# google-research/corenet

Hardware: AMD Instinct MI355X
Metric: voxels/sec fwd+bwd @128^3 (higher is better)
Workload: dtype bf16x3 (the convolutions of decoder stages 3-6 and the encoder's 3x3 convolutions -- forward of stages 4-5, data gradient of all -- multiply operands split into two bf16 terms: three bf16 MFMAs per product, fp32 accumulation, 16 mantissa bits, ~3e-6 relative per layer; tensors, everything else and t

## Files before the change

### corenet_amd/_lib.py

```python
from __future__ import annotations

import ctypes as C
import os
from typing import Optional

import torch as t

_HERE = os.path.dirname(os.path.abspath(__file__))
TOOLS_LIB_PATH = os.path.join(os.path.dirname(_HERE), "tools", "_build", "libcorenet_hip_tools.so")
PROBE_LIB_PATH = os.path.join(os.path.dirname(_HERE), "tools", "_build", "libcrn_probe.so")
LIB_PATH = os.environ.get("CORENET_HIP_LIB", TOOLS_LIB_PATH if os.environ.get("CRN_TOOLS_LIB") == "1" else
                          os.path.join(_HERE, "lib", "libcorenet_hip.so"))

c_i32p = C.POINTER(C.c_int32)
c_f32p = C.c_void_p
vp = C.c_void_p
i64 = C.c_int64
i32 = C.c_int
f32 = C.c_float
sz = C.c_size_t


class CrnTapBoxes(C.Structure):
  _fields_ = [("n_groups", C.c_int32), ("c_groups", C.c_int32), ("n_box", (C.c_int8 * 6) * 8),
# ... 104 lines not shown
    "crn_scatter_f32": [vp, vp, vp, i64, i32, vp],
    "crn_bias_grad": [vp, i32, i32, i64, i64, vp, i32, vp, sz, vp],
    "crn_batch_renorm_stats": [vp, i32, i32, i64, i64, i32, vp, vp, vp, vp, vp, f32, f32, i32,
                               vp, vp, vp, vp, sz, vp],
    "crn_batch_renorm_stats_tail": [vp, i32, i32, i64, i64, vp, vp, vp, vp, vp, f32, f32, i32, vp, vp, vp, vp, sz,
                                    vp, vp, vp, i64, vp, i64, vp, i64, i32, vp, i32, vp],
    "crn_batch_renorm_bwd_head": [vp, i64, vp, i64, vp, i64, vp, i64, vp, i64, i32, i32, i64, vp, vp, vp, vp, vp, i64,
                                  vp, vp, i32, vp, i32, vp, sz, vp, i32, vp],
    "crn_batch_renorm_bwd": [vp, i64, vp, i64, i32, i32, i64, i32, i32, vp, vp, vp, vp, vp, i64,
                             vp, vp, i32, vp, i32, vp, sz, vp],
    "crn_affine_add_relu": [vp, vp, vp, vp, vp, vp, i32, i32, i64, i64, i64, vp, i64, vp, i64, i32, vp],
    "crn_relu_bwd_add": [vp, vp, vp, i32, i32, i64, i64, i64, i64, vp, i64, vp],
    "crn_preprocess_caffe": [vp, i32, i32, i32, vp, vp],
    "crn_stem_conv_fwd": [vp, i32, i32, i32, vp, vp, vp, vp, sz, vp],
    "crn_stem_conv_wgrad": [vp, i32, i32, i32, vp, vp, vp],
    "crn_batch_renorm_finalize": [vp, i32, i32, C.c_double, vp, vp, vp, vp, vp, f32, f32, vp, vp, vp, vp],
    "crn_bn_relu_maxpool_fwd": [vp, vp, vp, i32, i32, i32, i32, vp, vp, vp],
    "crn_bn_relu_maxpool_bwd": [vp, vp, i32, i32, i32, i32, vp, vp],
    "crn_relu_mean_fwd": [vp, i32, i32, i64, i64, vp, vp],
    "crn_relu_mean_bwd": [vp, vp, i32, i32, i64, i64, vp, i64, i32, vp],
    "crn_linear_fwd": [vp, vp, vp, i32, i32, i32, vp, i32, vp],
    "crn_linear_bwd": [vp, vp, vp, i32, i32, i32, i32, vp, vp, vp, vp],
    "crn_stride2_gather": [vp, vp, i32, i32, i32, i32, i32, i32, vp],
    "crn_stride2_scatter": [vp, vp, i32, i32, i32, i32, i32, i32, vp],
    "crn_fill_offset_channels": [vp, i32, i64, i64, i32, vp, vp],
    "crn_decoder_inputs": [vp, vp, i32, i32, C.POINTER(C.c_float), vp, vp, vp],
    "crn_ray_sample_fwd": [vp, i64, i64, i64, i32, i32, i32, i32, vp, vp, vp, i64, i32, i32, i32, vp],
    "crn_ray_sample_bwd": [vp, i64, i32, i32, i32, i32, i32, vp, vp, vp, i64, i32, i32, i32, vp],
    "crn_ray_sample_fwd_idx": [vp, i64, i64, i64, i32, i32, i32, i32, vp, vp, vp, i64, i32, i32, i32, vp, vp],
    "crn_ray_project": [vp, vp, i32, i32, i32, i32, i32, i32, vp, vp],
# ... 193 lines not shown
```

### corenet_amd/backend.py

```python
from __future__ import annotations

import ctypes as C
from typing import Optional

import torch as t

from corenet_amd import _lib
from corenet_amd._lib import CrnInTransform, CrnView, ptr
from corenet_amd.views import View, space_to_depth_view, view_of

_DTYPE_CODE = {t.float32: 0, t.uint8: 1, t.int32: 2, t.float64: 3, t.int64: 4, t.int16: 5, t.int8: 6}


def _cview(v: View) -> CrnView:
  base = v.storage.data_ptr() + 4 * (v.offset - v.storage.storage_offset())
  c = v.__dict__.get("_crn")
  if c is None or c[0] != base:
    c = (base, CrnView(base, v.B, v.C, v.D, v.H, v.W, v.sB, v.sC, ptr(v.chan_off), v.sD, v.sH, v.sW))
    object.__setattr__(v, "_crn", c)
  return c[1]


class Transform:
  __slots__ = ("scale", "shift", "pre_relu", "post_relu")
# ... 333 lines not shown
  def relu_bwd_add(self, dy, y_pre, dy2, B, Cn, S, sB_dy, sB_pre, sB_dy2, dx, sB_dx):
    self.lib.crn_relu_bwd_add(ptr(dy), ptr(y_pre), ptr(dy2), B, Cn, S, sB_dy, sB_pre, sB_dy2,
                              ptr(dx), sB_dx, _lib.stream())

  def preprocess(self, img_u8, out):
    B, _, H, W = img_u8.shape
    self.lib.crn_preprocess_caffe(ptr(img_u8), B, H, W, ptr(out), _lib.stream())

  def maxpool_fwd(self, x, scale, shift, B, Cn, H, W, y, argmax):
    self.lib.crn_bn_relu_maxpool_fwd(ptr(x), ptr(scale), ptr(shift), B, Cn, H, W, ptr(y), ptr(argmax),
                                     _lib.stream())

  def maxpool_bwd(self, dy, argmax, B, Cn, H, W, dx):
    self.lib.crn_bn_relu_maxpool_bwd(ptr(dy), ptr(argmax), B, Cn, H, W, ptr(dx), _lib.stream())

  def relu_mean_fwd(self, x_pre, B, Cn, S, sB, avg):
    self.lib.crn_relu_mean_fwd(ptr(x_pre), B, Cn, S, sB, ptr(avg), _lib.stream())

  def relu_mean_bwd(self, x_pre, davg, B, Cn, S, sB, dx, sB_dx, accumulate=False):
    self.lib.crn_relu_mean_bwd(ptr(x_pre), ptr(davg), B, Cn, S, sB, ptr(dx), sB_dx, int(accumulate),
                               _lib.stream())

  def linear_fwd(self, x, w, bias, B, K, N, y, ldy):
    self.lib.crn_linear_fwd(ptr(x), ptr(w), ptr(bias), B, K, N, ptr(y), ldy, _lib.stream())

  def linear_bwd(self, x, w, dy, lddy, B, K, N, dx, dw, db):
    self.lib.crn_linear_bwd(ptr(x), ptr(w), ptr(dy), lddy, B, K, N, ptr(dx), ptr(dw), ptr(db),
                            _lib.stream())

  def stride2_gather(self, x, y):
# ... 202 lines not shown
```

### corenet_amd/build.py

```python
import os
import subprocess
import sys
from concurrent.futures import ThreadPoolExecutor

HERE = os.path.dirname(os.path.abspath(__file__))
CSRC = os.path.join(HERE, "csrc")
LIBDIR = os.path.join(HERE, "lib")
LIB = os.path.join(LIBDIR, "libcorenet_hip.so")
SOURCES = ["conv_igemm.hip", "splitk.hip", "conv_bf3.hip", "conv_e2d.hip", "batch_renorm.hip", "ray_sample.hip", "misc_ops.hip", "losses.hip", "fill_voxels.hip",
           "voxelize.hip", "comm_rccl.hip", "stem_conv.hip", "convt_par.hip", "fill_voxels_cpu.cpp", "marching_cubes.hip",
           "marching_cubes_cpu.cpp", "render.hip", "render_cpu.cpp", "point_metrics.hip", "point_metrics_cpu.cpp",
           "eval_labels.hip", "eval_labels_cpu.cpp", "voxel_components.hip", "voxel_components_cpu.cpp",
           "voxel_distance.hip", "voxel_distance_cpu.cpp", "voxel_visibility.hip", "voxel_visibility_cpu.cpp",
           "voxel_overlap.hip", "voxel_overlap_cpu.cpp"]
CONV_CONFIGS = [(8, 1), (4, 2), (4, 1), (2, 4), (2, 2), (2, 1), (1, 4), (1, 2), (1, 1)]
FLAGS = ["--offload-arch=gfx950", "-O3", "-std=c++17", "-fPIC", "-munsafe-fp-atomics",
         "-ffp-contract=off", "-Wno-unused-result"]


HOST_FLAGS = ["-O3", "-std=c++17", "-fPIC", "-ffp-contract=off", "-pthread"]


def _stale(obj, src):
  if not os.path.exists(obj):
    return True
  m = os.path.getmtime(obj)
  deps = [src, os.path.join(CSRC, "crn_common.h"), os.path.join(CSRC, "splitk.h"), os.path.join(CSRC, "conv_kernels.h"), os.path.join(CSRC, "bf3_common.h"),
          os.path.join(CSRC, "mc_tables.h"), os.path.join(CSRC, "marching_cubes_common.h"),
          os.path.join(CSRC, "render_common.h"), os.path.join(CSRC, "point_metrics_common.h"),
          os.path.join(CSRC, "eval_labels_common.h"), os.path.join(CSRC, "voxel_components_common.h"),
          os.path.join(CSRC, "voxel_distance_common.h"), os.path.join(CSRC, "voxel_visibility_common.h"),
          os.path.join(CSRC, "voxel_overlap_common.h"),
          os.path.join(HERE, "..", "include", "corenet_hip.h")]
  return any(os.path.getmtime(d) > m for d in deps)


def build(verbose=True, force=False):
  os.makedirs(LIBDIR, exist_ok=True)
  hipcc = os.environ.get("HIPCC", "/opt/rocm/bin/hipcc")
  objs, jobs = [], []
  for s in SOURCES:
    src = os.path.join(CSRC, s)
    obj = os.path.join(LIBDIR, os.path.splitext(s)[0] + ".o")
    objs.append(obj)
    if force or _stale(obj, src):
      flags = FLAGS if s.endswith(".hip") else HOST_FLAGS
      jobs.append([hipcc] + flags + ["-c", src, "-o", obj])
# ... 64 lines not shown
```

### corenet_amd/csrc/batch_renorm.hip

```cpp
#include "crn_common.h"
#include <cstdlib>
#include <algorithm>
#include <type_traits>

namespace {

constexpr int kThreads = 256;

struct Slice { int64_t s0, s1; };
__device__ __forceinline__ Slice block_slice(int64_t S) {
  int64_t chunk = (S + gridDim.x - 1) / gridDim.x;
  chunk = (chunk + 3) & ~(int64_t)3;
  Slice r;
  r.s0 = (int64_t)blockIdx.x * chunk;
  r.s1 = min(S, r.s0 + chunk);
  return r;
}

template <bool VEC, typename F4, typename F1>
__device__ __forceinline__ void for_slice(Slice sl, F4 f4, F1 f1) {
  if (VEC) {
#pragma unroll 4
    for (int64_t s = sl.s0 + (int64_t)threadIdx.x * 4; s + 3 < sl.s1; s += (int64_t)kThreads * 4) f4(s);
    const int64_t nfull = (sl.s1 > sl.s0) ? ((sl.s1 - sl.s0) & ~(int64_t)3) : 0;
// ... 259 lines not shown
        if (tail.y) {
          if (tail.relu) {
#pragma unroll
            for (int i = 0; i < 4; ++i) q[i] = fmaxf(q[i], 0.f);
          }
          *reinterpret_cast<f32x4*>(tail.y + (int64_t)b * tail.sBy + o) = q;
          int64_t o2;
          if (tail.y2 && bn_stride2_offset(c, s4, tail.W, tail.W2, tail.H2, o2))
            *reinterpret_cast<f32x2*>(tail.y2 + (int64_t)b * tail.sBy2 + o2) = (f32x2){q[0], q[2]};
        }
      }
    }
  }
}

struct BnBwdChannel { float sc, sh, mu, rstd; };
__device__ __forceinline__ BnBwdChannel bn_bwd_channel(int c, int C, const float* scale, const float* shift, const float* saved) {
  return BnBwdChannel{scale[c], shift[c], saved[c], saved[C + c]};
}

__device__ __forceinline__ void bn_bwd_acc(float x, float g, int pre_relu, int post_relu, BnBwdChannel ch, double& s1, double& s2) {
  if (pre_relu) x = fmaxf(x, 0.f);
  if (post_relu && !(x * ch.sc + ch.sh > 0.f)) g = 0.f;
  s1 += (double)g;
  s2 += (double)g * (double)((x - ch.mu) * ch.rstd);
}

__device__ __forceinline__ float bn_bwd_dx(float xr, float g, int pre_relu, int post_relu, BnBwdChannel ch, float k, float mg, float mgx) {
  const float x = pre_relu ? fmaxf(xr, 0.f) : xr;
  if (post_relu && !(x * ch.sc + ch.sh > 0.f)) g = 0.f;
  float o = k * (g - mg - (x - ch.mu) * ch.rstd * mgx);
  if (pre_relu && !(xr > 0.f)) o = 0.f;
  return o;
}

struct BnAffineGrad { float dg, db; };
__device__ __forceinline__ BnAffineGrad bn_bwd_close(double s1, double s2, double count, float r, float d, float* sm) {
  sm[0] = (float)(s1 / count); sm[1] = (float)(s2 / count);
  return BnAffineGrad{(float)(r * s2 + d * s1), (float)s1};
}
__device__ __forceinline__ void bn_bwd_store_grad(BnAffineGrad g, int c, float* dgamma, float* dbeta, int accumulate) {
  if (accumulate) { dgamma[c] += g.dg; dbeta[c] += g.db; } else { dgamma[c] = g.dg; dbeta[c] = g.db; }
}

__device__ __forceinline__ float bn_block_sum_f32(float v, float* redf) {
  const float w = crn_wave_sum(v);
  if ((threadIdx.x & 63) == 0) redf[threadIdx.x >> 6] = w;
  __syncthreads();
  float tsum = 0.f;
  if (threadIdx.x == 0)
    for (int i = 0; i < kThreads / 64; ++i) tsum += redf[i];
  return tsum;
}

struct BnHead { const float* g; int64_t sBg; const float* act; int64_t sBact; const float* g2; int64_t sBg2;
                const float* gc; int64_t sBgc; int W, W2, H2; };
template <int NV, bool HEAD = false>
__global__ __launch_bounds__(kThreads) void bn_owner_bwd_reg_kernel(
    const float* x, int64_t sBx, const float* dy, int64_t sBdy, int B, int S4, int C, int pre_relu,
// ... 85 lines not shown
    int post_relu, const float* scale, const float* shift, const float* saved, double* ws, float* dsum,
    int ndsum, const float* part, int splits) {
  __shared__ double red[kThreads / 64];
  const int c = blockIdx.y, b = blockIdx.z;
  if (dsum && c < ndsum && blockIdx.x == 0 && b == 0 && threadIdx.x == 0) dsum[c] = 0.f;
  const float* px = x + (int64_t)b * sBx + (int64_t)c * S;
  const BnPendingRow<PEND> pg = bn_pending_row<PEND>(dy, sBdy, part, splits, gridDim.z, C, S, b, c);
  const BnBwdChannel ch = bn_bwd_channel(c, C, scale, shift, saved);
  double s1 = 0.0, s2 = 0.0;
  auto one = [&](float xv, float gv) { bn_bwd_acc(xv, gv, pre_relu, post_relu, ch, s1, s2); };
  for_slice<VEC>(block_slice(S),
                 [&](int64_t s) { const f32x4 a = *reinterpret_cast<const f32x4*>(px + s);
                                  const f32x4 g = pg.at4(s);
                                  one(a.x, g.x); one(a.y, g.y); one(a.z, g.z); one(a.w, g.w); },
                 [&](int64_t s) { one(px[s], pg.at1(s)); });
  const double t1 = crn_block_sum(s1, red);
  const double t2 = crn_block_sum(s2, red);
  if (threadIdx.x == 0) {
    const int nparts = gridDim.x * gridDim.z;
    double* o = ws + ((int64_t)c * nparts + (int64_t)b * gridDim.x + blockIdx.x) * 2;
    o[0] = t1; o[1] = t2;
  }
}

template <bool VEC>
__global__ __launch_bounds__(kThreads) void bn_bwd_apply_kernel(
    const float* x, int64_t sBx, const float* dy, int64_t sBdy, int64_t S, int C, int pre_relu,
    int post_relu, const float* gamma, const float* scale, const float* shift, const float* saved,
    const double* ws, int nparts, double count, float* dx, int64_t sBdx, float* dgamma,
    float* dbeta, int accumulate, float* dsum, int ndsum) {
// ... 487 lines not shown
  float* const dsum_det = (dsum && ndsum > 0 && crn_deterministic()) ? dsum : nullptr;
  if (dsum_det && ws_bytes < (size_t)ndsum * ns * B * sizeof(double)) return CRN_ENOMEM;
  { const int rcf = crn_splitk_flush(st); if (rcf != CRN_OK) return rcf; }
  dim3 grid(ns, C, B);
  if (dsum_det) dsum = nullptr;
  with_bool(vec_ok(S, {sB_x, sB_dy, sB_dx}, {x, dy, dx}), [&](auto vec) {
    hipLaunchKernelGGL(bn_bwd_apply_kernel<decltype(vec)::value>, grid, dim3(kThreads), 0, st, x, sB_x, dy, sB_dy, S, C,
                       pre_relu, 0, gamma, scale, shift, saved, ws, nparts,
                       (double)B * (double)S, dx, sB_dx, dgamma, dbeta, accumulate, dsum, ndsum);
  });
  CRN_CHECK_LAUNCH();
  if (dsum_det) return bias_grad_ordered(dx, B, ndsum, S, sB_dx, ns, dsum_det, 0, ws, ws_bytes, st);
  return CRN_OK;
}

extern "C" int crn_batch_renorm_bwd_head(const float* x, int64_t sB_x, float* dy, int64_t sB_dy,
                                         const float* g, int64_t sB_g, const float* act, int64_t sB_act,
                                         const float* g2, int64_t sB_g2,
                                         int B, int C, int64_t S, const float* gamma, const float* scale,
                                         const float* shift, const float* saved, float* dx, int64_t sB_dx,
                                         float* dgamma, float* dbeta, int accumulate, float* dsum, int ndsum,
                                         double* ws, size_t ws_bytes, const float* g_compact, int W, crnStream stream) {
  if (!g || !act || !dy) return CRN_EINVAL;
  if (g_compact && (W < 1 || S % W || sB_g != (int64_t)C * S)) return CRN_EINVAL;
  const int H = g_compact ? (int)(S / W) : 0, H2 = (H + 1) / 2, W2 = (W + 1) / 2;
  const BnHead head{g, sB_g, act, sB_act, g2, sB_g2, g_compact, (int64_t)C * H2 * W2, W, W2, H2};
  return bn_bwd_impl(x, sB_x, dy, sB_dy, B, C, S, 0, 0, gamma, scale, shift, saved, dx, sB_dx, dgamma, dbeta,
                     accumulate, dsum, ndsum, ws, ws_bytes, stream, &head);
}

// ... 54 lines not shown
```

### corenet_amd/csrc/misc_ops.hip

```cpp
#include "crn_common.h"
#include <cstdlib>
#include <algorithm>
#include <cmath>

namespace {

__global__ void preprocess_kernel(const uint8_t* img, int64_t HW, float* out, int64_t total) {
  const int64_t e = blockIdx.x * (int64_t)blockDim.x + threadIdx.x;
  if (e >= total) return;
  const int64_t s = e % HW;
  const int c = (int)((e / HW) % 3);
  const int64_t b = e / (3 * HW);
  const float mean = c == 0 ? 103.939f : (c == 1 ? 116.779f : 123.68f);
  out[e] = (float)img[(b * 3 + (2 - c)) * HW + s] + mean;
}

__global__ void bn_relu_maxpool_fwd_kernel(const float* x, const float* scale, const float* shift,
                                           int C, int H, int W, int Ho, int Wo, float* y,
                                           int32_t* argmax, int64_t total) {
  const int64_t e = blockIdx.x * (int64_t)blockDim.x + threadIdx.x;
  if (e >= total) return;
  const int ow = (int)(e % Wo);
  const int oh = (int)((e / Wo) % Ho);
  const int64_t bc = e / ((int64_t)Wo * Ho);
// ... 15 lines not shown
    const float v = in ? fmaxf(raw[t9] * sc + sh, 0.f) : 0.f;
    const int idx = in ? ih * W + iw : -1;
    if (v > best) { best = v; bi = idx; }
  }
  y[e] = best;
  argmax[e] = (best > 0.f) ? bi : -1;
}

__global__ void bn_relu_maxpool_bwd_kernel(const float* dy, const int32_t* argmax, int H, int W,
                                           int Ho, int Wo, float* dx, int64_t total) {
  const int64_t e = blockIdx.x * (int64_t)blockDim.x + threadIdx.x;
  if (e >= total) return;
  const int iw = (int)(e % W);
  const int ih = (int)((e / W) % H);
  const int64_t bc = e / ((int64_t)W * H);
  const int idx = ih * W + iw;
  const float* g = dy + bc * (int64_t)Ho * Wo;
  const int32_t* am = argmax + bc * (int64_t)Ho * Wo;
  float s = 0.f;
  int amv[4];
  float gv[4];
#pragma unroll
  for (int q = 0; q < 4; ++q) {
    const int oh = min(ih / 2 + (q >> 1), Ho - 1), ow = min(iw / 2 + (q & 1), Wo - 1);
    amv[q] = am[oh * Wo + ow];
    gv[q] = g[oh * Wo + ow];
  }
#pragma unroll
  for (int q = 0; q < 4; ++q) {
    const int oh = ih / 2 + (q >> 1), ow = iw / 2 + (q & 1);
    const bool in = oh <= (ih + 1) / 2 && ow <= (iw + 1) / 2 && oh < Ho && ow < Wo;
    if (in && amv[q] == idx) s += gv[q];
  }
  dx[e] = s;
}

__global__ void relu_mean_fwd_kernel(const float* x, int C, int64_t S, int64_t sB, float* avg, int BC) {
  const int wid = (blockIdx.x * blockDim.x + threadIdx.x) >> 6, lane = threadIdx.x & 63;
  if (wid >= BC) return;
  const int b = wid / C, c = wid % C;
  const float* p = x + (int64_t)b * sB + (int64_t)c * S;
  double s = 0.0;
  for (int64_t i = lane; i < S; i += 64) s += (double)fmaxf(p[i], 0.f);
  s = crn_wave_sum(s);
  if (lane == 0) avg[wid] = (float)(s / (double)S);
}

__global__ void relu_mean_bwd_kernel(const float* x, const float* davg, int C, int64_t S, int64_t sB,
                                     float* dx, int64_t sBdx, int accumulate, int64_t total) {
// ... 535 lines not shown
```

### corenet_amd/csrc/stem_conv.hip

```cpp
#include "crn_common.h"
#include <cstdlib>
#include <algorithm>

namespace {

constexpr int kTH = 4, kTW = 32;
constexpr int kPH = 2 * kTH + 5;
constexpr int kPWf = 72;
constexpr int kPWg = 80;
constexpr int kKR = 3 * 7 * 8;
constexpr int kWP = 80;
constexpr int kDP = 84;
constexpr int kThreads = 256;

struct StemGeom {
  const float* img; const float* w; const float* bias; float* y; double* ws;
  const float* dy; float* dw;
  int B, H, W, H1, W1, tilesH, tilesW, ntiles;
};

__device__ __forceinline__ int packed_row(int c, int kh, int kw) {
  const int rh = (kh + 1) & 1, zh = (kh + 1) >> 1, rw = (kw + 1) & 1, zw = (kw + 1) >> 1;
  return (c * 4 + rh * 2 + rw) * 16 + zh * 4 + zw;
}

__device__ __forceinline__ void tile_of(const StemGeom& g, int tile, int& b, int& oh0, int& ow0) {
  const int tw = tile % g.tilesW; tile /= g.tilesW;
  const int th = tile % g.tilesH; b = tile / g.tilesH;
  oh0 = th * kTH; ow0 = tw * kTW;
}

template <int PW, int NE>
__device__ __forceinline__ void patch_load(const StemGeom& g, int b, int oh0, int ow0, int tid, float (&pv)[NE]) {
// ... 96 lines not shown
    for (int nb = 0; nb < 4; ++nb) {
      red[(wave * 64 + nb * 16 + i16) * 2 + 0] = s1[nb];
      red[(wave * 64 + nb * 16 + i16) * 2 + 1] = s2[nb];
    }
  }
  __syncthreads();
  if (tid < 64) {
    double a = 0.0, q = 0.0;
#pragma unroll
    for (int w = 0; w < 4; ++w) { a += (double)red[(w * 64 + tid) * 2]; q += (double)red[(w * 64 + tid) * 2 + 1]; }
    double* o = g.ws + ((int64_t)tid * gridDim.x + blockIdx.x) * 2;
    o[0] = a; o[1] = q;
  }
}

__global__ __launch_bounds__(kThreads) void stem_wgrad_kernel(StemGeom g) {
  __shared__ float pl[3 * kPH * kPWg];
  __shared__ float dl[kTH * kTW * kDP];
  crn_kernarg_touch(g);
  const int tid = threadIdx.x, lane = tid & 63, wave = tid >> 6, i16 = lane & 15, kk = lane >> 4;
  constexpr int NMB = (kKR + 15) / 16;
  int abase[NMB];
#pragma unroll
  for (int mb = 0; mb < NMB; ++mb) {
    const int T = min(mb * 16 + i16, kKR - 1);
    const int ck = T >> 3, kw = T & 7, c = ck / 7, kh = ck - c * 7;
    abase[mb] = (c * kPH + kh) * kPWg + kw + 2 * kk;
  }
  const int bbase = kk * kDP + wave * 16 + i16;
  f32x4 acc[NMB];
#pragma unroll
  for (int mb = 0; mb < NMB; ++mb) acc[mb] = (f32x4){0.f, 0.f, 0.f, 0.f};
  constexpr int NPE = (3 * kPH * kPWg + kThreads - 1) / kThreads;
  constexpr int NDV = kTH * kTW * 64 / 4 / kThreads;
  for (int tile = blockIdx.x; tile < g.ntiles; tile += gridDim.x) {
    int b, oh0, ow0;
    tile_of(g, tile, b, oh0, ow0);
    float pv[NPE];
    f32x4 dv[NDV];
    patch_load<kPWg>(g, b, oh0, ow0, tid, pv);
#pragma unroll
    for (int j = 0; j < NDV; ++j) {
      const int f = tid + j * kThreads;
      const int n = (f >> 9) * 16 + (f & 15), q4 = (f >> 4) & 31;
      const int oh = oh0 + (q4 >> 3), ow = ow0 + (q4 & 7) * 4;
      dv[j] = (oh < g.H1 && ow < g.W1) ? *reinterpret_cast<const f32x4*>(g.dy + ((int64_t)(b * 64 + n) * g.H1 + oh) * g.W1 + ow)
                                       : (f32x4){0.f, 0.f, 0.f, 0.f};
    }
    __syncthreads();
    patch_store<kPWg>(pl, tid, pv);
#pragma unroll
    for (int j = 0; j < NDV; ++j) {
      const int f = tid + j * kThreads;
      const int n = (f >> 9) * 16 + (f & 15), q4 = (f >> 4) & 31;
      float* d = dl + (q4 * 4) * kDP + n;
#pragma unroll
      for (int i = 0; i < 4; ++i) d[i * kDP] = dv[j][i];
    }
    __syncthreads();
#pragma unroll
    for (int q = 0; q < kTH * kTW / 4; ++q) {
      const int pr = q >> 3, qc = q & 7;
// ... 2 lines not shown
#pragma unroll
      for (int mb = 0; mb < NMB; ++mb)
        acc[mb] = __builtin_amdgcn_mfma_f32_16x16x4f32(pl[abase[mb] + ao], bv, acc[mb], 0, 0, 0);
    }
  }
  const int n = wave * 16 + i16;
#pragma unroll
  for (int mb = 0; mb < NMB; ++mb) {
#pragma unroll
    for (int r = 0; r < 4; ++r) {
      const int T = mb * 16 + kk * 4 + r;
      const int ck = T >> 3, kw = T & 7, c = ck / 7, kh = ck - c * 7;
      if (T < kKR && kw < 7) atomicAdd(g.dw + (int64_t)packed_row(c, kh, kw) * 64 + n, acc[mb][r]);
    }
  }
}

bool stem_shape_ok(int B, int H, int W) {
  return B >= 1 && H >= 8 && W >= 8 && (H & 1) == 0 && (W & 7) == 0 && (int64_t)B * H * W < ((int64_t)1 << 30);
}
StemGeom stem_geom(int B, int H, int W) {
  StemGeom g{};
  g.B = B; g.H = H; g.W = W; g.H1 = H / 2; g.W1 = W / 2;
  g.tilesH = crn_cdiv(g.H1, kTH); g.tilesW = crn_cdiv(g.W1, kTW);
  g.ntiles = B * g.tilesH * g.tilesW;
  return g;
}
}

extern "C" size_t crn_stem_conv_parts(int B, int H, int W) {
// ... 11 lines not shown
  if (stats_ws && ws_bytes < (size_t)64 * g.ntiles * 2 * sizeof(double)) return CRN_ENOMEM;
  hipLaunchKernelGGL(stem_fwd_kernel, dim3((unsigned)g.ntiles), dim3(kThreads), 0, (hipStream_t)stream, g);
  CRN_CHECK_LAUNCH();
  return CRN_OK;
}

extern "C" int crn_stem_conv_wgrad(const float* img, int B, int H, int W, const float* dy, float* dw_packed,
                                   crnStream stream) {
  CRN_ENTRY(stream);
  if (!img || !dy || !dw_packed || !stem_shape_ok(B, H, W)) return CRN_EINVAL;
  if (((uintptr_t)dy) & 15) return CRN_EINVAL;
  if (crn_deterministic()) return CRN_EINVAL;
  StemGeom g = stem_geom(B, H, W);
  g.img = img; g.dy = dy; g.dw = dw_packed;
  const int blocks = std::max(1, std::min(g.ntiles, 256));
  hipLaunchKernelGGL(stem_wgrad_kernel, dim3((unsigned)blocks), dim3(kThreads), 0, (hipStream_t)stream, g);
  CRN_CHECK_LAUNCH();
  return CRN_OK;
}
```

### corenet_amd/model/engine.py

```python
from __future__ import annotations

import dataclasses
import os
from typing import Dict, List, Optional, Tuple

import numpy as np
import torch as t

from corenet_amd import _lib
from corenet_amd import views as V
from corenet_amd.backend import Transform
from corenet_amd.model import conv_geometry as G

IMAGE_HW = (256, 256)


def check_image_hw(hw):
  H, W = int(hw[0]), int(hw[1])
  if H < 32 or W < 32 or H % 4 or W % 4 or H * W > 4096 * 4096:
    raise ValueError(f"corenet_amd.CoreNet: image batch of {H}x{W} pixels; this engine takes H and W that are multiples of 4 and >= 32 "
                     f"(256x256 in every shipped config)")
  return H, W
BN_EPS = 1e-3
BN_MOMENTUM = 0.01
# ... 547 lines not shown

def _no_exchange(grads: t.Tensor):
  """Bucket hook of a step without a gradient exchange."""


class Plan:

  def __init__(self, eng: Engine, B: int, hw=IMAGE_HW):
    self.eng, self.B = eng, B
    H, W = check_image_hw(hw)
    self.hw = (H, W)
    self.stem_hw = (H // 2, W // 2)
    parts = int(eng.be.lib.crn_stem_conv_parts(B, H, W)) if hasattr(eng.be, "stem_conv_fwd") else 0
    self.stem_fast = 0 < parts <= 4096
    self.dec_stats_fused = hasattr(eng.be, "conv_fwd_stats")
    self.pool_hw = (H // 4, W // 4)
    self.be = eng.be
    self.generation = 0
    self.graphs = {}
    self.eager_steps = 0
    self.eval_graph = None
    self.eval_eager = 0
    self._views = {}
    dev = eng.device
    self.dev = dev
    f = lambda *shape: t.zeros(*shape, dtype=eng.dtype, device=dev)
    self.in_image = t.zeros(B, 3, H, W, dtype=t.uint8, device=dev)
    self.in_v2s = f(B, 4, 4)
    self.in_off = f(B, 3)
    self.img = f(B, 3, H, W)
# ... 209 lines not shown
    g = cv.fwd
    math = self._math(cv, "wgrad")
    if self.stem_fast and cv.name == "encoder.stage1.conv.":
      math = "stem"
    if (self.eng.encoder_e2d and g.window in ((1, 1, 1), (1, 3, 3)) and self._wg2d_shape_ok(dy, g.window)
        and (cv.name.startswith("encoder.stage") and not cv.name.startswith("encoder.stage1")
             or cv.name.startswith("decoder.rt_skip"))):
      math = "bf16x3_2d"
    if cv.ct_kind == "par" and math == "bf16x3":
      math = "ct_par"
    return math

  def _launch_wgrad(self, cv: Conv, x: V.View, tr, dy: V.View, math: str, kw: dict):
    g = cv.fwd
    with _lib.roctx_range("wgrad " + cv.name):
      self.be.conv_wgrad(x, tr, dy, cv.gwf, g.npad, g.window, g.pad_lo, False, boxes=(g.n_boxes, g.c_boxes), math=math, **kw)

  def _wgrad(self, cv: Conv, x: V.View, tr, dy: V.View, here: bool = False):
    math = self._wgrad_math(cv, dy)
    kw = self._ximg_kw(math)
    if here:
      return self._launch_wgrad(cv, x, tr, dy, math, kw)
    if not self.overlap:
      return self._timed("wgrad " + cv.name, lambda: self._launch_wgrad(cv, x, tr, dy, math, kw))
    if cv.name.startswith("encoder."):
      self._wg_pending.append((cv, x, tr, dy, math, kw))
      return
    if self._handed_over:
      self._handed_over = False
      self._side_i = max(self._side_i, 1)
      ev = None
    else:
      ev = self._next_handover_event()
    with self._on_side(after=ev):
      self._launch_wgrad(cv, x, tr, dy, math, kw)
# ... 339 lines not shown
      t.cuda.current_stream().wait_event(self._skip_bwd_done)
    f5, g5 = self.feat["stage5"], self.gfeat["stage5"]
    last = self.blocks[-1]
    S5 = f5.shape[2] * f5.shape[3]
    be.relu_mean_bwd(f5, self.gavg, B, 2048, S5, f5.stride(0), last.gpre, 2048 * S5, False)
    be.affine_add_relu(last.gpre, None, None, g5, None, None, B, 2048, S5, 2048 * S5, g5.stride(0),
                       None, 0, last.gpre, 2048 * S5, False)
    g_in = None
    for blk in reversed(self.blocks):
      g_in = self._block_bwd(blk, g_in)
      self._flush_wgrads()
      if blk.prefix in GRAD_BUCKET_LABELS:
        self._grads_ready(blk.prefix, grad_hook)
    b1 = bn["encoder.stage1_part2.bn."]
    H1, W1 = self.stem_hw
    be.maxpool_bwd(g_in, self.p1_arg, B, 64, H1, W1, self.gy1)
    cs = cv["encoder.stage1.conv."]
    self._bn_bwd(b1, self.y1, self.gy1, self.gy1b, H1 * W1, False, False, bias_of=cs)
    self._wgrad(cs, self.s2d(self.img, 3, (1, 2, 2)), None, self.vw(self.gy1b))
    self._grads_ready("", grad_hook)
    self._join_side()
    if grad_hook is None:
      be.copy_tiles(eng.gpacked, eng.store.grads, eng.unpack_tiles, reverse=True)

  def _ray_bwd(self, k: int, g_out: t.Tensor):
    d, gm = self.dec[k], self.gsmap[k]
    ro, (hh, ww) = 2 * d.r, self.skip_hw[k]
    if self.ray_idx is not None:
      self.be.ray_sample_bwd_idx(g_out[:, d.cout:], g_out.stride(0), self.B, self.eng.skip_ch[k], ro, ro, ro,
                                 self.ray_idx[k], gm, gm.stride(0), hh, ww, False)
      return
    self.be.ray_sample_bwd(g_out[:, d.cout:], g_out.stride(0), self.B, self.eng.skip_ch[k], ro, ro, ro,
                           self.layer_mats[k - 2], self.offset, gm, gm.stride(0), hh, ww, False)

# ... 66 lines not shown
```

### include/corenet_hip.h

```cpp
#ifndef CORENET_HIP_H_
#define CORENET_HIP_H_

#include <stddef.h>
#include <stdint.h>

#ifdef __cplusplus
extern "C" {
#endif

#define CRN_OK 0
#define CRN_EINVAL (-1)
#define CRN_ENOMEM (-2)
#define CRN_ENOCONV (-3)

typedef void* crnStream;

typedef struct {
  float* base;
  int32_t B, C, D, H, W;
  int64_t sB, sC;
  const int32_t* chan_off;
  int32_t sD, sH, sW;
} crnView;

// ... 214 lines not shown

int crn_affine_add_relu(const float* x, const float* scale, const float* shift,
                        const float* r, const float* rscale, const float* rshift,
                        int B, int C, int64_t S, int64_t sB_x, int64_t sB_r,
                        float* y_pre, int64_t sB_pre, float* y, int64_t sB_y,
                        int relu, crnStream s);

int crn_relu_bwd_add(const float* dy, const float* y_pre, const float* dy2,
                     int B, int C, int64_t S, int64_t sB_dy, int64_t sB_pre, int64_t sB_dy2,
                     float* dx, int64_t sB_dx, crnStream s);

size_t crn_stem_conv_parts(int B, int H, int W);
int crn_stem_conv_fwd(const float* img, int B, int H, int W, const float* w_packed, const float* bias,
                      float* y, double* stats_ws , size_t ws_bytes, crnStream s);
int crn_stem_conv_wgrad(const float* img, int B, int H, int W, const float* dy, float* dw_packed, crnStream s);
int crn_batch_renorm_finalize(const double* ws, int nparts, int C, double count,
                              const float* gamma, const float* beta, float* running_mean, float* running_var,
                              const int64_t* nbt, float eps, float momentum,
                              float* scale, float* shift, float* saved, crnStream s);

int crn_preprocess_caffe(const uint8_t* img, int B, int H, int W, float* out, crnStream s);
int crn_bn_relu_maxpool_fwd(const float* x, const float* scale, const float* shift,
                            int B, int C, int H, int W, float* y, int32_t* argmax, crnStream s);
int crn_bn_relu_maxpool_bwd(const float* dy, const int32_t* argmax, int B, int C, int H, int W,
                            float* dx_bn , crnStream s);
int crn_relu_mean_fwd(const float* x_pre, int B, int C, int64_t S, int64_t sB, float* avg, crnStream s);
int crn_linear_fwd(const float* x, const float* w, const float* bias, int B, int K, int N,
                   float* y, int ldy, crnStream s);
int crn_linear_bwd(const float* x, const float* w, const float* dy, int lddy, int B, int K, int N,
                   float* dx, float* dw, float* db, crnStream s);
// ... 252 lines not shown
```

Measured before the change: 1.208 billion.

## Fuse stem maxpool backward with BN sums and BN-dx into stem wgrad

Replaces the three-step stem backward tail (maxpool backward, batch-renorm backward, stem weight-gradient) with two kernels. The maxpool backward now also accumulates the per-channel BN reduction sums. The stem wgrad kernel reduces those sums, applies the BN dx transform on the fly and also writes dgamma/dbeta and the bias gradient. This removes one full-resolution pass and the gy1b intermediate, at the cost of more complex kernels, an extra x load inside wgrad, and a non-deterministic path that is skipped under deterministic mode.

Result: no change. 1.198 billion (-0.9%).

```diff
diff --git a/corenet_amd/_lib.py b/corenet_amd/_lib.py
--- a/corenet_amd/_lib.py
+++ b/corenet_amd/_lib.py
@@ -142,6 +142,8 @@
     "crn_preprocess_caffe": [vp, i32, i32, i32, vp, vp],
     "crn_stem_conv_fwd": [vp, i32, i32, i32, vp, vp, vp, vp, sz, vp],
     "crn_stem_conv_wgrad": [vp, i32, i32, i32, vp, vp, vp],
+    "crn_maxpool_bwd_bn_sums": [vp, vp, i32, i32, i32, i32, vp, vp, vp, vp, vp, vp, i32, vp, sz, C.POINTER(C.c_int), vp],
+    "crn_stem_conv_wgrad_bn": [vp, i32, i32, i32, vp, vp, vp, vp, vp, sz, i32, vp, vp, vp, vp, i32, vp],
     "crn_batch_renorm_finalize": [vp, i32, i32, C.c_double, vp, vp, vp, vp, vp, f32, f32, vp, vp, vp, vp],
     "crn_bn_relu_maxpool_fwd": [vp, vp, vp, i32, i32, i32, i32, vp, vp, vp],
     "crn_bn_relu_maxpool_bwd": [vp, vp, i32, i32, i32, i32, vp, vp],
diff --git a/corenet_amd/backend.py b/corenet_amd/backend.py
--- a/corenet_amd/backend.py
+++ b/corenet_amd/backend.py
@@ -371,6 +371,24 @@
   def maxpool_bwd(self, dy, argmax, B, Cn, H, W, dx):
     self.lib.crn_bn_relu_maxpool_bwd(ptr(dy), ptr(argmax), B, Cn, H, W, ptr(dx), _lib.stream())
 
+  def maxpool_bwd_bn_sums(self, dy, argmax, B, Cn, H, W, x, scale, shift, saved, g, dsum=None, ndsum=0):
+    ws, n = self._bn_ws(Cn, x.device)
+    nparts = C.c_int(0)
+    self.lib.crn_maxpool_bwd_bn_sums(ptr(dy), ptr(argmax), B, Cn, H, W, ptr(x), ptr(scale), ptr(shift), ptr(saved), ptr(g),
+                                     ptr(dsum), int(ndsum), ptr(ws), n, C.byref(nparts), _lib.stream())
+    return ws, n, nparts.value
+
+  def stem_conv_wgrad_bn(self, img, gy, y, gamma, saved, sums, dw, dgamma, dbeta, dsum=None, ndsum=0) -> bool:
+    B, _, H, W = img.shape
+    ws, n, nparts = sums
+    rc = self.lib._crn_stem_conv_wgrad_bn(ptr(img), B, H, W, ptr(gy), ptr(y), ptr(gamma), ptr(saved), ptr(ws), n, nparts,
+                                          ptr(dw), ptr(dgamma), ptr(dbeta), ptr(dsum), int(ndsum), _lib.stream())
+    if rc == -1:
+      return False
+    if rc != 0:
+      raise _lib.HipError(f"crn_stem_conv_wgrad_bn failed with status {rc}")
+    return True
+
   def relu_mean_fwd(self, x_pre, B, Cn, S, sB, avg):
     self.lib.crn_relu_mean_fwd(ptr(x_pre), B, Cn, S, sB, ptr(avg), _lib.stream())
 
diff --git a/corenet_amd/build.py b/corenet_amd/build.py
--- a/corenet_amd/build.py
+++ b/corenet_amd/build.py
@@ -30,7 +30,7 @@
           os.path.join(CSRC, "render_common.h"), os.path.join(CSRC, "point_metrics_common.h"),
           os.path.join(CSRC, "eval_labels_common.h"), os.path.join(CSRC, "voxel_components_common.h"),
           os.path.join(CSRC, "voxel_distance_common.h"), os.path.join(CSRC, "voxel_visibility_common.h"),
-          os.path.join(CSRC, "voxel_overlap_common.h"),
+          os.path.join(CSRC, "voxel_overlap_common.h"), os.path.join(CSRC, "bn_bwd_common.h"),
           os.path.join(HERE, "..", "include", "corenet_hip.h")]
   return any(os.path.getmtime(d) > m for d in deps)
 
diff --git a/corenet_amd/csrc/batch_renorm.hip b/corenet_amd/csrc/batch_renorm.hip
--- a/corenet_amd/csrc/batch_renorm.hip
+++ b/corenet_amd/csrc/batch_renorm.hip
@@ -1,4 +1,5 @@
 #include "crn_common.h"
+#include "bn_bwd_common.h"
 #include <cstdlib>
 #include <algorithm>
 #include <type_traits>
@@ -297,35 +298,6 @@
   }
 }
 
-struct BnBwdChannel { float sc, sh, mu, rstd; };
-__device__ __forceinline__ BnBwdChannel bn_bwd_channel(int c, int C, const float* scale, const float* shift, const float* saved) {
-  return BnBwdChannel{scale[c], shift[c], saved[c], saved[C + c]};
-}
-
-__device__ __forceinline__ void bn_bwd_acc(float x, float g, int pre_relu, int post_relu, BnBwdChannel ch, double& s1, double& s2) {
-  if (pre_relu) x = fmaxf(x, 0.f);
-  if (post_relu && !(x * ch.sc + ch.sh > 0.f)) g = 0.f;
-  s1 += (double)g;
-  s2 += (double)g * (double)((x - ch.mu) * ch.rstd);
-}
-
-__device__ __forceinline__ float bn_bwd_dx(float xr, float g, int pre_relu, int post_relu, BnBwdChannel ch, float k, float mg, float mgx) {
-  const float x = pre_relu ? fmaxf(xr, 0.f) : xr;
-  if (post_relu && !(x * ch.sc + ch.sh > 0.f)) g = 0.f;
-  float o = k * (g - mg - (x - ch.mu) * ch.rstd * mgx);
-  if (pre_relu && !(xr > 0.f)) o = 0.f;
-  return o;
-}
-
-struct BnAffineGrad { float dg, db; };
-__device__ __forceinline__ BnAffineGrad bn_bwd_close(double s1, double s2, double count, float r, float d, float* sm) {
-  sm[0] = (float)(s1 / count); sm[1] = (float)(s2 / count);
-  return BnAffineGrad{(float)(r * s2 + d * s1), (float)s1};
-}
-__device__ __forceinline__ void bn_bwd_store_grad(BnAffineGrad g, int c, float* dgamma, float* dbeta, int accumulate) {
-  if (accumulate) { dgamma[c] += g.dg; dbeta[c] += g.db; } else { dgamma[c] = g.dg; dbeta[c] = g.db; }
-}
-
 __device__ __forceinline__ float bn_block_sum_f32(float v, float* redf) {
   const float w = crn_wave_sum(v);
   if ((threadIdx.x & 63) == 0) redf[threadIdx.x >> 6] = w;
@@ -441,6 +413,42 @@
                                   const f32x4 g = pg.at4(s);
                                   one(a.x, g.x); one(a.y, g.y); one(a.z, g.z); one(a.w, g.w); },
                  [&](int64_t s) { one(px[s], pg.at1(s)); });
+  const double t1 = crn_block_sum(s1, red);
+  const double t2 = crn_block_sum(s2, red);
+  if (threadIdx.x == 0) {
+    const int nparts = gridDim.x * gridDim.z;
+    double* o = ws + ((int64_t)c * nparts + (int64_t)b * gridDim.x + blockIdx.x) * 2;
+    o[0] = t1; o[1] = t2;
+  }
+}
+
+template <bool VEC>
+__global__ __launch_bounds__(kThreads) void maxpool_bwd_bn_sums_kernel(
+    const float* __restrict__ dyp, const int32_t* __restrict__ argmax, int H, int W, int Ho, int Wo, const float* __restrict__ x,
+    int C, const float* __restrict__ scale, const float* __restrict__ shift, const float* __restrict__ saved, float* __restrict__ g,
+    double* __restrict__ ws, float* __restrict__ dsum, int ndsum) {
+  __shared__ double red[kThreads / 64];
+  const int c = blockIdx.y, b = blockIdx.z;
+  const int64_t S = (int64_t)H * W, So = (int64_t)Ho * Wo, bc = (int64_t)b * C + c;
+  if (dsum && c < ndsum && blockIdx.x == 0 && b == 0 && threadIdx.x == 0) dsum[c] = 0.f;
+  const float* __restrict__ px = x + bc * S;
+  float* __restrict__ pg = g + bc * S;
+  const float* __restrict__ gp = dyp + bc * So;
+  const int32_t* __restrict__ am = argmax + bc * So;
+  const BnBwdChannel ch = bn_bwd_channel(c, C, scale, shift, saved);
+  double s1 = 0.0, s2 = 0.0;
+  const bool rows4 = (W & 3) == 0;
+  auto pool = [&](int s) { const int ih = s / W; return crn_maxpool_bwd_at(gp, am, ih, s - ih * W, W, Ho, Wo); };
+  auto one = [&](float xv, float gv) { bn_bwd_acc(xv, gv, 0, 0, ch, s1, s2); };
+  for_slice<VEC>(block_slice(S),
+                 [&](int64_t s64) { const int s = (int)s64;
+                                    const f32x4 a = *reinterpret_cast<const f32x4*>(px + s);
+                                    float gv[4];
+                                    if (rows4) { const int ih = s / W; crn_maxpool_bwd_at4(gp, am, ih, s - ih * W, W, Ho, Wo, gv); }
+                                    else { gv[0] = pool(s); gv[1] = pool(s + 1); gv[2] = pool(s + 2); gv[3] = pool(s + 3); }
+                                    *reinterpret_cast<f32x4*>(pg + s) = (f32x4){gv[0], gv[1], gv[2], gv[3]};
+                                    one(a.x, gv[0]); one(a.y, gv[1]); one(a.z, gv[2]); one(a.w, gv[3]); },
+                 [&](int64_t s64) { const int s = (int)s64; const float gv = pool(s); pg[s] = gv; one(px[s], gv); });
   const double t1 = crn_block_sum(s1, red);
   const double t2 = crn_block_sum(s2, red);
   if (threadIdx.x == 0) {
@@ -958,6 +966,26 @@
   return CRN_OK;
 }
 
+extern "C" int crn_maxpool_bwd_bn_sums(const float* dy, const int32_t* argmax, int B, int C, int H, int W, const float* x,
+                                       const float* scale, const float* shift, const float* saved, float* g, float* dsum,
+                                       int ndsum, double* ws, size_t ws_bytes, int* nparts_out, crnStream stream) {
+  CRN_ENTRY(stream);
+  hipStream_t st = (hipStream_t)stream;
+  if (B < 1 || C < 1 || H < 1 || W < 1 || B > 64 || (int64_t)H * W >= ((int64_t)1 << 31)) return CRN_EINVAL;
+  if (!dy || !argmax || !x || !scale || !shift || !saved || !g || !ws || !nparts_out) return CRN_EINVAL;
+  const int64_t S = (int64_t)H * W;
+  const int Ho = (H + 2 - 3) / 2 + 1, Wo = (W + 2 - 3) / 2 + 1;
+  const int ns = nsplit_for(S, C, B);
+  if (ws_bytes < (size_t)C * ns * B * 2 * sizeof(double)) return CRN_ENOMEM;
+  with_bool(vec_ok(S, {C * S}, {x, g}), [&](auto vec) {
+    hipLaunchKernelGGL(maxpool_bwd_bn_sums_kernel<decltype(vec)::value>, dim3(ns, C, B), dim3(kThreads), 0, st, dy, argmax, H, W,
+                       Ho, Wo, x, C, scale, shift, saved, g, ws, dsum, ndsum);
+  });
+  CRN_CHECK_LAUNCH();
+  *nparts_out = ns * B;
+  return CRN_OK;
+}
+
 extern "C" int crn_batch_renorm_bwd_head(const float* x, int64_t sB_x, float* dy, int64_t sB_dy,
                                          const float* g, int64_t sB_g, const float* act, int64_t sB_act,
                                          const float* g2, int64_t sB_g2,
diff --git a/corenet_amd/csrc/bn_bwd_common.h b/corenet_amd/csrc/bn_bwd_common.h
--- /dev/null
+++ b/corenet_amd/csrc/bn_bwd_common.h
@@ -0,0 +1,76 @@
+#pragma once
+#include "crn_common.h"
+
+struct BnBwdChannel { float sc, sh, mu, rstd; };
+__device__ __forceinline__ BnBwdChannel bn_bwd_channel(int c, int C, const float* scale, const float* shift, const float* saved) {
+  return BnBwdChannel{scale[c], shift[c], saved[c], saved[C + c]};
+}
+
+__device__ __forceinline__ void bn_bwd_acc(float x, float g, int pre_relu, int post_relu, BnBwdChannel ch, double& s1, double& s2) {
+  if (pre_relu) x = fmaxf(x, 0.f);
+  if (post_relu && !(x * ch.sc + ch.sh > 0.f)) g = 0.f;
+  s1 += (double)g;
+  s2 += (double)g * (double)((x - ch.mu) * ch.rstd);
+}
+
+__device__ __forceinline__ float bn_bwd_dx(float xr, float g, int pre_relu, int post_relu, BnBwdChannel ch, float k, float mg, float mgx) {
+  const float x = pre_relu ? fmaxf(xr, 0.f) : xr;
+  if (post_relu && !(x * ch.sc + ch.sh > 0.f)) g = 0.f;
+  float o = k * (g - mg - (x - ch.mu) * ch.rstd * mgx);
+  if (pre_relu && !(xr > 0.f)) o = 0.f;
+  return o;
+}
+
+struct BnAffineGrad { float dg, db; };
+__device__ __forceinline__ BnAffineGrad bn_bwd_close(double s1, double s2, double count, float r, float d, float* sm) {
+  sm[0] = (float)(s1 / count); sm[1] = (float)(s2 / count);
+  return BnAffineGrad{(float)(r * s2 + d * s1), (float)s1};
+}
+__device__ __forceinline__ void bn_bwd_store_grad(BnAffineGrad g, int c, float* dgamma, float* dbeta, int accumulate) {
+  if (accumulate) { dgamma[c] += g.dg; dbeta[c] += g.db; } else { dgamma[c] = g.dg; dbeta[c] = g.db; }
+}
+
+__device__ __forceinline__ float crn_maxpool_bwd_at(const float* g, const int32_t* am, int ih, int iw, int W, int Ho, int Wo) {
+  const int idx = ih * W + iw;
+  float s = 0.f;
+  int amv[4];
+  float gv[4];
+#pragma unroll
+  for (int q = 0; q < 4; ++q) {
+    const int oh = min(ih / 2 + (q >> 1), Ho - 1), ow = min(iw / 2 + (q & 1), Wo - 1);
+    amv[q] = am[oh * Wo + ow];
+    gv[q] = g[oh * Wo + ow];
+  }
+#pragma unroll
+  for (int q = 0; q < 4; ++q) {
+    const int oh = ih / 2 + (q >> 1), ow = iw / 2 + (q & 1);
+    const bool in = oh <= (ih + 1) / 2 && ow <= (iw + 1) / 2 && oh < Ho && ow < Wo;
+    if (in && amv[q] == idx) s += gv[q];
+  }
+  return s;
+}
+
+__device__ __forceinline__ void crn_maxpool_bwd_at4(const float* __restrict__ g, const int32_t* __restrict__ am, int ih, int iw,
+                                                    int W, int Ho, int Wo, float (&out)[4]) {
+  int amc[2][3];
+  float gc[2][3];
+#pragma unroll
+  for (int r = 0; r < 2; ++r)
+#pragma unroll
+    for (int c = 0; c < 3; ++c) {
+      const int o = min(ih / 2 + r, Ho - 1) * Wo + min(iw / 2 + c, Wo - 1);
+      amc[r][c] = am[o]; gc[r][c] = g[o];
+    }
+#pragma unroll
+  for (int j = 0; j < 4; ++j) {
+    const int w = iw + j, idx = ih * W + w;
+    float s = 0.f;
+#pragma unroll
+    for (int q = 0; q < 4; ++q) {
+      const int oh = ih / 2 + (q >> 1), ow = w / 2 + (q & 1);
+      const bool in = oh <= (ih + 1) / 2 && ow <= (w + 1) / 2 && oh < Ho && ow < Wo;
+      if (in && amc[q >> 1][(j >> 1) + (q & 1)] == idx) s += gc[q >> 1][(j >> 1) + (q & 1)];
+    }
+    out[j] = s;
+  }
+}
diff --git a/corenet_amd/csrc/misc_ops.hip b/corenet_amd/csrc/misc_ops.hip
--- a/corenet_amd/csrc/misc_ops.hip
+++ b/corenet_amd/csrc/misc_ops.hip
@@ -1,4 +1,5 @@
 #include "crn_common.h"
+#include "bn_bwd_common.h"
 #include <cstdlib>
 #include <algorithm>
 #include <cmath>
@@ -53,25 +54,7 @@
   const int iw = (int)(e % W);
   const int ih = (int)((e / W) % H);
   const int64_t bc = e / ((int64_t)W * H);
-  const int idx = ih * W + iw;
-  const float* g = dy + bc * (int64_t)Ho * Wo;
-  const int32_t* am = argmax + bc * (int64_t)Ho * Wo;
-  float s = 0.f;
-  int amv[4];
-  float gv[4];
-#pragma unroll
-  for (int q = 0; q < 4; ++q) {
-    const int oh = min(ih / 2 + (q >> 1), Ho - 1), ow = min(iw / 2 + (q & 1), Wo - 1);
-    amv[q] = am[oh * Wo + ow];
-    gv[q] = g[oh * Wo + ow];
-  }
-#pragma unroll
-  for (int q = 0; q < 4; ++q) {
-    const int oh = ih / 2 + (q >> 1), ow = iw / 2 + (q & 1);
-    const bool in = oh <= (ih + 1) / 2 && ow <= (iw + 1) / 2 && oh < Ho && ow < Wo;
-    if (in && amv[q] == idx) s += gv[q];
-  }
-  dx[e] = s;
+  dx[e] = crn_maxpool_bwd_at(dy + bc * (int64_t)Ho * Wo, argmax + bc * (int64_t)Ho * Wo, ih, iw, W, Ho, Wo);
 }
 
 __global__ void relu_mean_fwd_kernel(const float* x, int C, int64_t S, int64_t sB, float* avg, int BC) {
diff --git a/corenet_amd/csrc/stem_conv.hip b/corenet_amd/csrc/stem_conv.hip
--- a/corenet_amd/csrc/stem_conv.hip
+++ b/corenet_amd/csrc/stem_conv.hip
@@ -1,4 +1,5 @@
 #include "crn_common.h"
+#include "bn_bwd_common.h"
 #include <cstdlib>
 #include <algorithm>
 
@@ -17,6 +18,8 @@
   const float* img; const float* w; const float* bias; float* y; double* ws;
   const float* dy; float* dw;
   int B, H, W, H1, W1, tilesH, tilesW, ntiles;
+  const float* x1; const float* gamma; const float* saved; const double* bws; int nparts, bG, bLg; double count;
+  float* dgamma; float* dbeta; float* dsum; int ndsum;
 };
 
 __device__ __forceinline__ int packed_row(int c, int kh, int kw) {
@@ -143,11 +146,63 @@
   }
 }
 
+template <bool BN>
 __global__ __launch_bounds__(kThreads) void stem_wgrad_kernel(StemGeom g) {
   __shared__ float pl[3 * kPH * kPWg];
-  __shared__ float dl[kTH * kTW * kDP];
+  __shared__ __attribute__((aligned(16))) float dl[kTH * kTW * kDP];
+  __shared__ float chn[BN ? 64 * 5 : 1];
   crn_kernarg_touch(g);
   const int tid = threadIdx.x, lane = tid & 63, wave = tid >> 6, i16 = lane & 15, kk = lane >> 4;
+  if (BN) {
+    constexpr int kApplyThreads = 256;
+    float cg = 0.f, cmu = 0.f, crs = 0.f, cr = 0.f, cd = 0.f;
+    if (tid < 64) { cg = g.gamma[tid]; cmu = g.saved[tid]; crs = g.saved[64 + tid]; cr = g.saved[128 + tid]; cd = g.saved[192 + tid]; }
+    const int G = g.bG, per = 64 / G, slot = lane & (G - 1), grp = lane >> g.bLg;
+    double ra[16], rb[16];
+#pragma unroll
+    for (int r = 0; r < 16; ++r) ra[r] = rb[r] = 0.0;
+    for (int w0 = 0; w0 < kApplyThreads && w0 < g.nparts; w0 += 64) {
+      double q1[16], q2[16];
+#pragma unroll
+      for (int r = 0; r < 16; ++r) {
+        const int cw = r * per + grp, i = w0 + slot;
+        const bool ok = cw < 16 && i < g.nparts;
+        const double* wsc = g.bws + ((int64_t)(wave * 16 + (ok ? cw : 0)) * g.nparts + (ok ? i : 0)) * 2;
+        const double a = wsc[0], b = wsc[1];
+        q1[r] = ok ? 0.0 + a : 0.0; q2[r] = ok ? 0.0 + b : 0.0;
+      }
+      if (g.nparts > kApplyThreads) {
+#pragma unroll
+        for (int r = 0; r < 16; ++r) {
+          const double* wsc = g.bws + (int64_t)(wave * 16 + r) * g.nparts * 2;
+          for (int i = w0 + slot + kApplyThreads; i < g.nparts; i += kApplyThreads) { q1[r] += wsc[(int64_t)i * 2]; q2[r] += wsc[(int64_t)i * 2 + 1]; }
+        }
+      }
+#pragma unroll
+      for (int r = 0; r < 16; ++r) {
+        if (r * per < 16) {
+          for (int o = G >> 1; o > 0; o >>= 1) { q1[r] += __shfl_down(q1[r], o, 64); q2[r] += __shfl_down(q2[r], o, 64); }
+          ra[r] += q1[r]; rb[r] += q2[r];
+        }
+      }
+    }
+    double* csum = reinterpret_cast<double*>(dl);
+#pragma unroll
+    for (int r = 0; r < 16; ++r) {
+      const int cw = r * per + grp;
+      if (slot == 0 && cw < 16) { csum[(wave * 16 + cw) * 2] = ra[r]; csum[(wave * 16 + cw) * 2 + 1] = rb[r]; }
+    }
+    __syncthreads();
+    if (tid < 64) {
+      float* cp = chn + tid * 5;
+      const BnAffineGrad ag = bn_bwd_close(csum[tid * 2], csum[tid * 2 + 1], g.count, cr, cd, cp + 1);
+      cp[0] = cg * cr * crs;
+      cp[3] = cmu; cp[4] = crs;
+      if (blockIdx.x == 0) bn_bwd_store_grad(ag, tid, g.dgamma, g.dbeta, 0);
+    }
+    __syncthreads();
+  }
+  float lsum[4] = {0.f, 0.f, 0.f, 0.f};
   constexpr int NMB = (kKR + 15) / 16;
   int abase[NMB];
 #pragma unroll
@@ -166,15 +221,33 @@
     int b, oh0, ow0;
     tile_of(g, tile, b, oh0, ow0);
     float pv[NPE];
-    f32x4 dv[NDV];
+    f32x4 dv[NDV], xv[BN ? NDV : 1];
     patch_load<kPWg>(g, b, oh0, ow0, tid, pv);
 #pragma unroll
     for (int j = 0; j < NDV; ++j) {
       const int f = tid + j * kThreads;
       const int n = (f >> 9) * 16 + (f & 15), q4 = (f >> 4) & 31;
       const int oh = oh0 + (q4 >> 3), ow = ow0 + (q4 & 7) * 4;
-      dv[j] = (oh < g.H1 && ow < g.W1) ? *reinterpret_cast<const f32x4*>(g.dy + ((int64_t)(b * 64 + n) * g.H1 + oh) * g.W1 + ow)
-                                       : (f32x4){0.f, 0.f, 0.f, 0.f};
+      const bool ok = oh < g.H1 && ow < g.W1;
+      const int64_t at = ((int64_t)(b * 64 + n) * g.H1 + oh) * g.W1 + ow;
+      dv[j] = ok ? *reinterpret_cast<const f32x4*>(g.dy + at) : (f32x4){0.f, 0.f, 0.f, 0.f};
+      if (BN) xv[j] = ok ? *reinterpret_cast<const f32x4*>(g.x1 + at) : (f32x4){0.f, 0.f, 0.f, 0.f};
+    }
+    if (BN) {
+#pragma unroll
+      for (int j = 0; j < NDV; ++j) {
+        const int f = tid + j * kThreads;
+        const int n = (f >> 9) * 16 + (f & 15), q4 = (f >> 4) & 31;
+        const float* cp = chn + n * 5;
+        const BnBwdChannel ch{0.f, 0.f, cp[3], cp[4]};
+        if (oh0 + (q4 >> 3) < g.H1 && ow0 + (q4 & 7) * 4 < g.W1) {
+#pragma unroll
+          for (int i = 0; i < 4; ++i) {
+            dv[j][i] = bn_bwd_dx(xv[j][i], dv[j][i], 0, 0, ch, cp[0], cp[1], cp[2]);
+            lsum[j >> 1] += dv[j][i];
+          }
+        }
+      }
     }
     __syncthreads();
     patch_store<kPWg>(pl, tid, pv);
@@ -207,6 +280,17 @@
       if (T < kKR && kw < 7) atomicAdd(g.dw + (int64_t)packed_row(c, kh, kw) * 64 + n, acc[mb][r]);
     }
   }
+  if (!BN || !g.dsum) return;
+#pragma unroll
+  for (int q = 0; q < 4; ++q) { lsum[q] += __shfl_xor(lsum[q], 16); lsum[q] += __shfl_xor(lsum[q], 32); }
+  __syncthreads();
+  float* red = dl;
+  if (kk == 0) {
+#pragma unroll
+    for (int q = 0; q < 4; ++q) red[wave * 64 + q * 16 + i16] = lsum[q];
+  }
+  __syncthreads();
+  if (tid < 64 && tid < g.ndsum) atomicAdd(g.dsum + tid, red[tid] + red[64 + tid] + red[128 + tid] + red[192 + tid]);
 }
 
 bool stem_shape_ok(int B, int H, int W) {
@@ -248,7 +332,29 @@
   StemGeom g = stem_geom(B, H, W);
   g.img = img; g.dy = dy; g.dw = dw_packed;
   const int blocks = std::max(1, std::min(g.ntiles, 256));
-  hipLaunchKernelGGL(stem_wgrad_kernel, dim3((unsigned)blocks), dim3(kThreads), 0, (hipStream_t)stream, g);
+  hipLaunchKernelGGL(stem_wgrad_kernel<false>, dim3((unsigned)blocks), dim3(kThreads), 0, (hipStream_t)stream, g);
   CRN_CHECK_LAUNCH();
   return CRN_OK;
 }
+
+extern "C" int crn_stem_conv_wgrad_bn(const float* img, int B, int H, int W, const float* gy, const float* y,
+                                      const float* gamma, const float* saved, const double* sums_ws, size_t ws_bytes, int nparts,
+                                      float* dw_packed, float* dgamma, float* dbeta, float* dsum, int ndsum, crnStream stream) {
+  CRN_ENTRY(stream);
+  if (!img || !gy || !y || !gamma || !saved || !sums_ws || !dw_packed || !dgamma || !dbeta || !stem_shape_ok(B, H, W)) return CRN_EINVAL;
+  if ((((uintptr_t)gy) | ((uintptr_t)y)) & 15) return CRN_EINVAL;
+  if (nparts < 1 || ndsum < 0 || ndsum > 64) return CRN_EINVAL;
+  if (ws_bytes < (size_t)64 * nparts * 2 * sizeof(double)) return CRN_ENOMEM;
+  if (crn_deterministic()) return CRN_EINVAL;
+  StemGeom g = stem_geom(B, H, W);
+  g.img = img; g.dy = gy; g.dw = dw_packed;
+  g.x1 = y; g.gamma = gamma; g.saved = saved; g.bws = sums_ws; g.nparts = nparts;
+  while (g.bLg < 6 && (1 << g.bLg) < nparts) ++g.bLg;
+  g.bG = 1 << g.bLg;
+  g.count = (double)B * (double)g.H1 * (double)g.W1;
+  g.dgamma = dgamma; g.dbeta = dbeta; g.dsum = dsum; g.ndsum = ndsum;
+  const int blocks = std::max(1, std::min(g.ntiles, 256));
+  hipLaunchKernelGGL(stem_wgrad_kernel<true>, dim3((unsigned)blocks), dim3(kThreads), 0, (hipStream_t)stream, g);
+  CRN_CHECK_LAUNCH();
+  return CRN_OK;
+}
diff --git a/corenet_amd/model/engine.py b/corenet_amd/model/engine.py
--- a/corenet_amd/model/engine.py
+++ b/corenet_amd/model/engine.py
@@ -585,6 +585,9 @@
     parts = int(eng.be.lib.crn_stem_conv_parts(B, H, W)) if hasattr(eng.be, "stem_conv_fwd") else 0
     self.stem_fast = 0 < parts <= 4096
     self.dec_stats_fused = hasattr(eng.be, "conv_fwd_stats")
+    self.stem_tail_fused = (self.stem_fast and eng.decoder_math == "bf16x3" and hasattr(eng.be, "stem_conv_wgrad_bn")
+                            and hasattr(eng.be, "maxpool_bwd_bn_sums"))
+    self.stem_tail_on_main = True
     self.pool_hw = (H // 4, W // 4)
     self.be = eng.be
     self.generation = 0
@@ -824,11 +827,21 @@
   def _launch_wgrad(self, cv: Conv, x: V.View, tr, dy: V.View, math: str, kw: dict):
     g = cv.fwd
     with _lib.roctx_range("wgrad " + cv.name):
+      if math == "stem_bn":
+        b, sums = kw["stem_bn"]
+        if self.be.stem_conv_wgrad_bn(self.img, self.gy1, self.y1, b.gamma, b.saved, sums, cv.gwf, b.dgamma, b.dbeta,
+                                      dsum=cv.dbias, ndsum=cv.n_ref):
+          return
+        H1, W1 = self.stem_hw
+        self._bn_bwd(b, self.y1, self.gy1, self.gy1b, H1 * W1, False, False, bias_of=cv)
+        dy, math, kw = self.vw(self.gy1b), "stem", _NO_KW
       self.be.conv_wgrad(x, tr, dy, cv.gwf, g.npad, g.window, g.pad_lo, False, boxes=(g.n_boxes, g.c_boxes), math=math, **kw)
 
-  def _wgrad(self, cv: Conv, x: V.View, tr, dy: V.View, here: bool = False):
+  def _wgrad(self, cv: Conv, x: V.View, tr, dy: V.View, here: bool = False, stem_bn=None):
     math = self._wgrad_math(cv, dy)
     kw = self._ximg_kw(math)
+    if stem_bn is not None:
+      math, kw = "stem_bn", {"stem_bn": stem_bn}
     if here:
       return self._launch_wgrad(cv, x, tr, dy, math, kw)
     if not self.overlap:
@@ -1198,10 +1211,15 @@
         self._grads_ready(blk.prefix, grad_hook)
     b1 = bn["encoder.stage1_part2.bn."]
     H1, W1 = self.stem_hw
-    be.maxpool_bwd(g_in, self.p1_arg, B, 64, H1, W1, self.gy1)
     cs = cv["encoder.stage1.conv."]
-    self._bn_bwd(b1, self.y1, self.gy1, self.gy1b, H1 * W1, False, False, bias_of=cs)
-    self._wgrad(cs, self.s2d(self.img, 3, (1, 2, 2)), None, self.vw(self.gy1b))
+    if self.stem_tail_fused and not getattr(be, "_deterministic", False):
+      sums = be.maxpool_bwd_bn_sums(g_in, self.p1_arg, B, 64, H1, W1, self.y1, b1.scale, b1.shift, b1.saved, self.gy1,
+                                    dsum=cs.dbias, ndsum=cs.n_ref)
+      self._wgrad(cs, self.s2d(self.img, 3, (1, 2, 2)), None, self.vw(self.gy1), here=self.stem_tail_on_main, stem_bn=(b1, sums))
+    else:
+      be.maxpool_bwd(g_in, self.p1_arg, B, 64, H1, W1, self.gy1)
+      self._bn_bwd(b1, self.y1, self.gy1, self.gy1b, H1 * W1, False, False, bias_of=cs)
+      self._wgrad(cs, self.s2d(self.img, 3, (1, 2, 2)), None, self.vw(self.gy1b))
     self._grads_ready("", grad_hook)
     self._join_side()
     if grad_hook is None:
diff --git a/include/corenet_hip.h b/include/corenet_hip.h
--- a/include/corenet_hip.h
+++ b/include/corenet_hip.h
@@ -252,6 +252,12 @@
 int crn_stem_conv_fwd(const float* img, int B, int H, int W, const float* w_packed, const float* bias,
                       float* y, double* stats_ws , size_t ws_bytes, crnStream s);
 int crn_stem_conv_wgrad(const float* img, int B, int H, int W, const float* dy, float* dw_packed, crnStream s);
+int crn_maxpool_bwd_bn_sums(const float* dy, const int32_t* argmax, int B, int C, int H, int W, const float* x,
+                            const float* scale, const float* shift, const float* saved, float* g, float* dsum, int ndsum,
+                            double* sums_ws, size_t ws_bytes, int* nparts_out, crnStream s);
+int crn_stem_conv_wgrad_bn(const float* img, int B, int H, int W, const float* gy, const float* y, const float* gamma,
+                           const float* saved, const double* sums_ws, size_t ws_bytes, int nparts, float* dw_packed,
+                           float* dgamma, float* dbeta, float* dsum, int ndsum, crnStream s);
 int crn_batch_renorm_finalize(const double* ws, int nparts, int C, double count,
                               const float* gamma, const float* beta, float* running_mean, float* running_var,
                               const int64_t* nbt, float eps, float momentum,
```
